# dalek-cryptography/curve25519-dalek

Measured on AMD Instinct MI355X. Metric: MSM scalar-mults/sec (variable-base Pippenger MSM), higher is better.
Workload: dtype u32 limbs (radix 2^25.5), u64 accumulators

## Files before the change

### curve25519-dalek_amd/csrc/accum.hip

```cpp
#include <hip/hip_runtime.h>
#include <stdlib.h>
#define C25519_CHAIN 1
#include "devio.h"
#include "msm_internal.h"
#include "fe26x.h"
#include "msm_sort.h"
#include "mid_long.h"

namespace c25519 {

#if defined(__HIP_DEVICE_COMPILE__)
#define ge_madd_acc ge_madd_signed_p3_lockstep
#else
#define ge_madd_acc ge_madd_signed_p3
#endif

#ifndef C25519_ACC_WAVES
#define C25519_ACC_WAVES 3
#endif
__device__ __forceinline__ void accumulate_body(const u32 *__restrict__ pts, const u32 *__restrict__ sorted, const u32 *__restrict__ base,
             const u32 *__restrict__ perm, u64 count, u64 n, const msm_geom &g, u32 *__restrict__ buckets, int cont, u32 block, uint4 *stage) {
    const u64 tid = (u64)block * blockDim.x + threadIdx.x;
    const bool in_range = tid < count;
    const u64 gid = in_range ? perm[tid] : 0;
// ... 53 lines not shown
        if (active) acc = ge_madd_acc(acc, pts_from_q(q), neg);
#else
        if (active) {
            const u32 me = (u32)((int)e >> 31), flip = me ^ sgn;
            sgn = me;
            acc = ge_madd_lazy_p3_lockstep(acc, pts_from_q(q), flip);
        }
#endif
        e = e_next;
    }
#undef C25519_COOP_ISSUE
    if (!mine) return;
#if !defined(C25519_ACC_SIGN_SELECT) && defined(__HIP_DEVICE_COMPILE__)
    acc.X = fe_carry(feW(fe_cond_neg(acc.X, sgn))); acc.T = fe_carry(feW(fe_cond_neg(acc.T, sgn)));
#endif
    p40_store(buckets, gid, acc);
}
__global__ void __launch_bounds__(256) __attribute__((amdgpu_waves_per_eu(C25519_ACC_WAVES, C25519_ACC_WAVES)))
k_accumulate(const u32 *__restrict__ pts, const u32 *__restrict__ sorted, const u32 *__restrict__ base,
             const u32 *__restrict__ perm, u64 count, u64 n, msm_geom g, u32 *__restrict__ buckets, int cont) {
    __shared__ uint4 stage[(256 / 64) * 8 * 64];
    accumulate_body(pts, sorted, base, perm, count, n, g, buckets, cont, blockIdx.x, stage);
}
struct acc_long_args { const mid_item *items; const u32 *counters; u32 *seg_sums; u32 *long_done; u32 max_items, blocks; };
__global__ void __launch_bounds__(256) __attribute__((amdgpu_waves_per_eu(C25519_ACC_WAVES, C25519_ACC_WAVES)))
k_accumulate_long(const u32 *__restrict__ pts, const u32 *__restrict__ sorted, const u32 *__restrict__ base,
                  const u32 *__restrict__ perm, u64 count, u64 n, msm_geom g, u32 *__restrict__ buckets, acc_long_args L) {
    __shared__ uint4 stage[(256 / 64) * 8 * 64];
    if (blockIdx.x < L.blocks) {
        C25519_PRIO_LONG();
        mid_long_body<1>(pts, sorted, n, g, buckets, L.max_items, L.items, L.counters, L.seg_sums, L.long_done, blockIdx.x * 4u + (threadIdx.x >> 6), L.blocks * 4u);
        return;
    }
    accumulate_body(pts, sorted, base, perm, count, n, g, buckets, 0, blockIdx.x - L.blocks, stage);
}

}

const char *launch_accumulate(const uint32_t *pts, const uint32_t *sorted, const uint32_t *base, const uint32_t *perm, uint64_t count, uint64_t n, const c25519::msm_geom &g, uint32_t *buckets, int cont, hipStream_t st) {
    using namespace c25519;
    hipLaunchKernelGGL(k_accumulate, dim3((unsigned)((count + 255) / 256)), dim3(256), 0, st, pts, sorted, base, perm, count, n, g, buckets, cont);
    return "c25519::k_accumulate (lockstep field products, wave-cooperative gather)";
}
const char *launch_accumulate_long(const uint32_t *pts, const uint32_t *sorted, const uint32_t *base, const uint32_t *perm, uint64_t count, uint64_t n, const c25519::msm_geom &g, uint32_t *buckets,
                                   const void *items, const uint32_t *counters, uint32_t *seg_sums, uint32_t *long_done, uint32_t max_items, uint32_t long_blocks, hipStream_t st) {
    using namespace c25519;
    acc_long_args L = {(const mid_item *)items, counters, seg_sums, long_done, max_items, long_blocks};
    hipLaunchKernelGGL(k_accumulate_long, dim3((unsigned)((count + 255) / 256) + long_blocks), dim3(256), 0, st, pts, sorted, base, perm, count, n, g, buckets, L);
    return "c25519::k_accumulate_long (mid path: bucket lanes of k_accumulate behind the blocks of the over-long lists)";
}
```

### curve25519-dalek_amd/csrc/msm.hip

```cpp
#include <hip/hip_runtime.h>
#include <algorithm>
#include <stdio.h>
#include <stdlib.h>
#include <string.h>
#include <stdexcept>
#include <string>
#include <vector>
#include "../../include/c25519_hip.h"
#include "devio.h"
#include "sc_sha.h"
#include "sc28.h"
#include "kernels.h"
#include "ctx.h"
#include "msm_internal.h"
#include "msm_sort.h"
#include "host51.h"
#include "ffi.h"
#include "capi_util.h"
#include <functional>

using namespace c25519;

namespace c25519 {

// ... 402 lines not shown
    msm_layout(layout_terms ? layout_terms : n, g);
    for (int i = 0; i < reps; i++) {
        msm_plan pl;
        pl.bad_sticky = nullptr;
        int32_t r = msm_enqueue_sort(ctx, d_scalars, n, g, dslot(ctx, 0), nullptr, pl);
        if (r) return r;
    }
    HIPCHK(hipStreamSynchronize(ctx->stream));
    return C25519_OK;
}

static_assert(C25519_SLOT_U32 == MSM_MAX_WIN * 40 + 16, "slot layout");

int32_t msm_enqueue_acc(c25519_ctx *ctx, const msm_plan &pl, const uint32_t *d_pts, uint32_t *d_slot, hipEvent_t *ring, hipEvent_t wait_acc, bool cont, bool reduce,
                        const uint32_t *d_bad_sticky) {
    const msm_geom &g = pl.g;
    if (pl.n > (1ull << 25)) return bad_arg(ctx, "msm: internal error (a pass of more than 2^25 records)");
    if (pl.sort_stream && pl.sort_stream != ctx->stream) {
        HIPCHK(hipEventRecord(ctx->ev_sort, pl.sort_stream));
        HIPCHK(hipStreamWaitEvent(ctx->stream, ctx->ev_sort, 0));
    }
    hipStream_t st = ctx->stream;
    if (wait_acc) HIPCHK(hipStreamWaitEvent(st, wait_acc, 0));
    HIPCHK(hipEventRecord(ctx->ev_fork, st));
    HIPCHK(hipStreamWaitEvent(ctx->aux, ctx->ev_fork, 0));
    hipLaunchKernelGGL(k_long_segments, dim3(std::min<uint32_t>(pl.max_items, 2048u)), dim3(64), 0, ctx->aux, d_pts, pl.sorted, pl.n, g, pl.items, pl.counters, pl.max_items, pl.segs);
    hipLaunchKernelGGL(k_long_combine, dim3(std::min<uint32_t>(pl.max_long, 1024u)), dim3(64), 0, ctx->aux, pl.base, g, pl.counters, pl.max_items, pl.lgids, pl.lfirst, pl.segs, pl.buckets, cont ? 1 : 0);
    if (ring) HIPCHK(hipEventRecord(ring[0], st));
    static const int coop_reduce = C25519_KNOB("REDUCE_COOP", 1);
    const int groups = (g.ngroups > 1 && reduce && !cont && coop_reduce) ? g.ngroups : 1;
    static const int reduce_main = C25519_KNOB("REDUCE_MAIN", 1);
    const bool red_main = reduce_main && ctx->solo && reduce && !cont && groups == 1 && coop_reduce && !wait_acc;
    for (int q = 0; q < groups; q++) {
        const int k0 = groups > 1 ? g.gstart[q] : 0, k1 = groups > 1 ? g.gstart[q + 1] : g.nwin;
        ctx->kname[0] = launch_accumulate(d_pts, pl.sorted, pl.base, pl.perm + (size_t)k0 * g.half, (uint64_t)(k1 - k0) * g.half, pl.n, g, pl.buckets, cont ? 1 : 0, st);
        if (groups > 1) {
            HIPCHK(hipEventRecord(ctx->ev_grp[q], st));
            HIPCHK(hipStreamWaitEvent(ctx->aux, ctx->ev_grp[q], 0));
            launch_bucket_reduce4(pl.buckets, g, pl.nseg, pl.SW, d_slot, d_bad_sticky ? d_bad_sticky : pl.bad_ws, ctx->aux, k0, k1);
            HIPCHK(hipGetLastError());
        }
    }
    HIPCHK(hipEventRecord(ctx->ev_acc, st));
    if (ring) HIPCHK(hipEventRecord(ring[1], st));
    if (red_main) {
        HIPCHK(hipEventRecord(ctx->ev_join, ctx->aux));
        HIPCHK(hipStreamWaitEvent(st, ctx->ev_join, 0));
        launch_bucket_reduce4(pl.buckets, g, pl.nseg, pl.SW, d_slot, d_bad_sticky ? d_bad_sticky : pl.bad_ws, st);
        HIPCHK(hipGetLastError());
        if (ring) HIPCHK(hipEventRecord(ring[2], st));
        return C25519_OK;
    }
    if (reduce && groups == 1) HIPCHK(hipStreamWaitEvent(ctx->aux, ctx->ev_acc, 0));
    if (groups > 1) {
    } else if (reduce && coop_reduce) {
        launch_bucket_reduce4(pl.buckets, g, pl.nseg, pl.SW, d_slot, d_bad_sticky ? d_bad_sticky : pl.bad_ws, ctx->aux);
        HIPCHK(hipGetLastError());
    } else if (reduce) {
// ... 338 lines not shown
    if (!ahead) {
        if ((r = ctx_reserve(ctx, ctx->tmp_e, std::max(n, n_carve) * PTS_BYTES + 256))) return r;
        d_pts = (uint32_t *)ctx->tmp_e.p;
    } else d_pts = ahead->pts + ahead->offset * (PTS_BYTES / 4);
    hipEvent_t *ring = pass_ring(owner, ctx, 1);
    HIPCHK(hipEventRecord(ring[3], ctx->stream));
    HIPCHK(hipEventRecord(ctx->ev_fork, ctx->stream));
    static const int sweep_early = C25519_KNOB("SWEEP_EARLY", 1);
    const bool early = sweep_early && cont && !wait_in && terms > msm_small_max() && parity >= 0;
    hipEvent_t lists_free = nullptr;
    if (parity >= 0) {
        HIPCHK(hipEventRecord(ctx->ev_lists[parity & 1], ctx->stream));
        if (early) lists_free = sweep_early >= 2 ? ctx->ev_lists[(parity & 1) ^ 1] : ctx->ev_fork;
    }
    if (!early) HIPCHK(hipStreamWaitEvent(ctx->aux, ctx->ev_fork, 0));
    if (!cont && !ctx->direct_seq) slot_init(d_slot, terms, nullptr, ctx->stream, g.c);
    if (terms <= msm_small_max() && g.half <= 64 && g.nwin <= 64 && !cont && reduce && !ahead) {
        if (in_fmt == C25519_FMT_RAW160) return msm_small_pass(ctx, d_scalars, d_points, 0, n, g, d_slot, ring, nullptr, wait_acc);
        if ((r = prep_points(ctx, d_points, n, in_fmt, d_pts, 0, slot_flags(d_slot) + 1))) return r;
        return msm_small_pass(ctx, d_scalars, d_pts, 1, n, g, d_slot, ring, nullptr, wait_acc);
    }
    msm_plan pl;
    pl.bad_sticky = d_bad_sticky;
    static const int serial_sort = C25519_KNOB("PROFILE_SERIAL_SORT", 0);
    static const int sort_first = C25519_KNOB("SORT_FIRST", 0);
    const bool sorted_first = sort_first && !ahead && !serial_sort && !cont && !wait_in;
    if (sorted_first) {
        pl.ev_partition = nullptr;
        if ((r = msm_enqueue_sort(ctx, d_scalars, n, g, d_slot, ctx->aux, pl, nullptr, n_carve, lists_free, sweep_early >= 2 ? parity : -1))) return r;
        if (pl.ev_partition) HIPCHK(hipStreamWaitEvent(ctx->stream, pl.ev_partition, 0));
    }
    if (!ahead) { if ((r = prep_points(ctx, d_points, n, in_fmt, d_pts, 0, slot_flags(d_slot) + 1))) return r; }
    else if (ahead->launch) {
        if ((r = prep_points(ctx, d_points, ahead->n, in_fmt, ahead->pts, 0, slot_flags(d_slot) + 1))) return r;
        HIPCHK(hipEventRecord(ahead->done, ctx->stream));
    } else HIPCHK(hipStreamWaitEvent(ctx->stream, ahead->done, 0));
    if (serial_sort) { HIPCHK(hipEventRecord(ctx->ev_z, ctx->stream)); HIPCHK(hipStreamWaitEvent(ctx->aux, ctx->ev_z, 0)); }
    if (!sorted_first && (r = msm_enqueue_sort(ctx, d_scalars, n, g, d_slot, ctx->aux, pl, nullptr, n_carve, lists_free, sweep_early >= 2 ? parity : -1))) return r;
    if (cont && pl.buckets != ctx->cont_buckets) return bad_arg(ctx, "msm: internal error (the workspace of a continuing pass moved its buckets)");
    ctx->cont_buckets = pl.buckets;
    if ((r = msm_enqueue_acc(ctx, pl, d_pts, d_slot, ring, wait_acc, cont, reduce, d_bad_sticky))) return r;
    return C25519_OK;
}
typedef std::function<int32_t(uint64_t lo, uint64_t m, hipEvent_t *ready)> msm_fetch;
static int32_t msm_record_enqueue(c25519_ctx *ctx, const uint8_t *d_scalars, const uint8_t *d_points, uint64_t n, int in_fmt, uint32_t *d_record,
                                  const msm_fetch *fetch = nullptr, uint64_t pass_terms = 0) {
// ... 251 lines not shown
```

### curve25519-dalek_amd/csrc/msm_internal.h

```cpp
#pragma once
#include <hip/hip_runtime.h>
#include <stdint.h>
#include <stdlib.h>
#include "ge26.h"
#include "ctx.h"

#include "knobs.h"
namespace c25519 {
constexpr int MSM_MAX_WIN = 56;
constexpr int MSM_MAX_GROUPS = 4;
struct msm_geom { int c, nwin, half, first_unsigned, bps_log2; u32 long_cap; u32 addk[8]; unsigned char pos[MSM_MAX_WIN], wid[MSM_MAX_WIN], bps[MSM_MAX_WIN];
                  unsigned char ngroups, gstart[MSM_MAX_GROUPS + 1]; };
__host__ __device__ inline int msm_group_of(const msm_geom &g, int k) { int r = 0; for (int i = 1; i < g.ngroups; i++) r += k >= (int)g.gstart[i] ? 1 : 0; return r; }
struct msm_merged { int c, K; uint64_t ns; };
constexpr u32 LONG_CAP_MIN = 192;
constexpr u32 LONG_SEG = 1024;
}
namespace c25519 {
struct long_item;
static inline int red_lb_log2(int half) {
    static const int lb_min = [] { const int v = C25519_KNOB("RED_LB_MIN", 1); return v < 1 ? 1 : (v > 3 ? 3 : v); }();
    if (half <= 512) return 3;
    int lb = lb_min;
    while ((half >> (lb + 6)) > 64) lb++;
    return lb;
}
static inline int red_nseg(int half) { const int seg = 64 << red_lb_log2(half); return (half + seg - 1) / seg; }
constexpr int REC_TERMS_LO = 8, REC_TERMS_HI = 9, REC_PASSES = 10, REC_MAGIC = 11, REC_C = 12;
constexpr u32 REC_MAGIC_VALUE = 0x52503235u;
inline uint64_t msm_small_max() { static const uint64_t v = (uint64_t)C25519_KNOB("MSM_SMALL_MAX", 6143); return v; }
inline uint64_t verify_small_max() { static const uint64_t v = (uint64_t)C25519_KNOB("VERIFY_SMALL_MAX", 4095); return v < msm_small_max() ? v : msm_small_max(); }
inline uint64_t small_upload_max_terms() { static const uint64_t v = (uint64_t)C25519_KNOB_LL("VERIFY_STAGED_MAX", 32769); return v; }
}
static inline unsigned div_up64(uint64_t a, uint64_t b) { return (unsigned)((a + b - 1) / b); }
static inline uint32_t *slot_flags(uint32_t *slot) { return slot + c25519::MSM_MAX_WIN * 40; }
static inline uint32_t *dslot(c25519_ctx *ctx, int i) { return ctx->d_slots + (size_t)i * C25519_SLOT_U32; }
static inline const uint32_t *hslot(c25519_ctx *ctx, int i) { return (const uint32_t *)ctx->h_msm + (size_t)i * C25519_SLOT_U32; }
static inline uint32_t *drec(c25519_ctx *ctx) { return dslot(ctx, C25519_MAX_SLOTS); }
struct msm_plan {
    c25519::msm_geom g; uint64_t n, nb; int nseg; uint32_t max_items, max_long;
    uint32_t *base, *sorted, *buckets, *perm, *SW, *counters, *lgids, *lfirst, *segs, *bad_ws, *bad_sticky = nullptr; c25519::long_item *items;
    hipStream_t sort_stream;
    hipEvent_t ev_partition = nullptr;
};
void msm_sort_params(uint64_t n, c25519::msm_geom &g);
void msm_slice_params(c25519::msm_geom &g);
int32_t msm_enqueue_sort(c25519_ctx *ctx, const uint8_t *d_scalars, uint64_t n_scalars, const c25519::msm_geom &g, uint32_t *d_slot, hipStream_t sort_stream, msm_plan &pl,
                         const c25519::msm_merged *md = nullptr, uint64_t n_carve = 0, hipEvent_t lists_free = nullptr, int parity = -1);
struct msm_matrix_sort_args {
    const uint8_t *d_scalars; uint64_t n_scalars, n; int nchunk; bool use_part; int SL, PART_CHUNK, pchunks;
    uint16_t *D; uint32_t *counts, *P1, *cc, *bin_base, *flags, *totals, *ord_hist;
};
int32_t msm_matrix_sort_enqueue(c25519_ctx *ctx, const c25519::msm_geom &g, const c25519::msm_merged *md, msm_plan &pl, const msm_matrix_sort_args &a, hipStream_t st);
int32_t msm_enqueue_acc(c25519_ctx *ctx, const msm_plan &pl, const uint32_t *d_pts, uint32_t *d_slot, hipEvent_t *ring, hipEvent_t wait_acc, bool cont = false, bool reduce = true,
                        const uint32_t *d_bad_sticky = nullptr);
struct mid_run;
int32_t msm_enqueue(c25519_ctx *ctx, const uint8_t *d_scalars, uint64_t n, const uint32_t *d_pts, const c25519::msm_geom &g, uint32_t *d_slot, hipEvent_t *ring,
                    hipStream_t sort_stream, hipEvent_t wait_acc = nullptr, const struct mid_run *run = nullptr);
int32_t msm_small_enqueue(c25519_ctx *ctx, const uint8_t *d_scalars, const void *d_points, int src_fmt, uint64_t n, const c25519::msm_geom &g, uint32_t *d_slot, hipStream_t st);
c25519::ge_p3 host_p40(const uint32_t *t);
c25519::ge_p3 msm_horner(const uint32_t *cols, const c25519::msm_geom &g);
int32_t slots_collect(c25519_ctx *ctx, int count);
int32_t rec_collect(c25519_ctx *ctx);
void slot_init(uint32_t *d_slot, uint64_t terms, const uint32_t *d_pre, hipStream_t st, int c);
int32_t records_fold(const uint8_t *records, uint64_t count, c25519::ge_p3 &R, uint32_t flags[8], std::string *err);
struct pass_set { c25519_ctx *c[4]; int lanes; };
int32_t passes_begin(c25519_ctx *ctx, uint64_t passes, pass_set &ps);
int32_t passes_join(c25519_ctx *ctx, pass_set &ps);
hipEvent_t *pass_ring(c25519_ctx *owner, c25519_ctx *c, uint8_t kind);
void launch_merged_table(const uint8_t *in_raw, uint64_t ns, int c, int K, uint8_t *out_raw, hipStream_t st);
void launch_bucket_reduce4(const uint32_t *buckets, const c25519::msm_geom &g, int nseg, uint32_t *SW, uint32_t *d_slot, const uint32_t *bad_ws, hipStream_t st, int k0 = 0, int k1 = -1);
void msm_set_groups(c25519::msm_geom &g, int groups, int last);
namespace c25519 { struct reduce_publish { int on; uint32_t *host_flag; uint32_t seq, terms_lo, terms_hi, c; int hdr; const uint32_t *dev_flags; }; }
void launch_bucket_reduce_pub(const uint32_t *buckets, const c25519::msm_geom &g, int nseg, uint32_t *SW, uint32_t *out, const uint32_t *blockflags, int nflags, uint32_t *done_cnt,
                              const c25519::reduce_publish &pub, hipStream_t st);
void launch_order_place(const uint32_t *totals, uint64_t nb, const uint32_t *ord_hist, uint32_t *ord_cursor, uint32_t *perm, const c25519::msm_geom &g, hipStream_t st);
uint64_t msm_mid_max();
bool msm_mid_serves_terms(uint64_t n);
bool msm_mid_serves(uint64_t n, const c25519::msm_geom &g, bool prepared);
struct mid_run { hipStream_t stream; hipEvent_t recs_ready; const uint8_t *sign_z16; uint64_t sign_first, sign_count; };
int32_t msm_mid_enqueue(c25519_ctx *ctx, const uint8_t *d_scalars, const void *points, int src_fmt, uint64_t n, const c25519::msm_geom &g, uint32_t *d_slot, int hdr, uint64_t terms, hipEvent_t *ring,
                        const mid_run *run = nullptr);
void launch_apply_sign(uint32_t *pts, uint64_t dst0, const uint8_t *z16, uint64_t n, hipStream_t st);
void launch_prep_basepoint(uint32_t *pts, uint64_t dst, hipStream_t st);
void launch_record_sum(uint32_t *rec, const uint32_t *slots, int cnt, int nwin, int first, hipStream_t st);
const char *launch_accumulate(const uint32_t *pts, const uint32_t *sorted, const uint32_t *base, const uint32_t *perm, uint64_t count, uint64_t n, const c25519::msm_geom &g, uint32_t *buckets, int cont, hipStream_t st);
const char *launch_accumulate_long(const uint32_t *pts, const uint32_t *sorted, const uint32_t *base, const uint32_t *perm, uint64_t count, uint64_t n, const c25519::msm_geom &g, uint32_t *buckets,
                                   const void *items, const uint32_t *counters, uint32_t *seg_sums, uint32_t *long_done, uint32_t max_items, uint32_t long_blocks, hipStream_t st);
void msm_layout(uint64_t n, c25519::msm_geom &g, int cmax = 0, int c_exact = 0);
int32_t msm_core(c25519_ctx *ctx, const uint8_t *d_scalars, uint64_t n, const uint32_t *d_pts, c25519::ge_p3 &R);
void msm_merged_layout(uint64_t ns, c25519::msm_merged &m);
int32_t msm_merged_core(c25519_ctx *ctx, const uint8_t *d_scalars, uint64_t n, const c25519::msm_merged &m, const uint32_t *d_table, c25519::ge_p3 &R);
int32_t msm_merged_build(c25519_ctx *ctx, const uint8_t *d_points, uint64_t ns, int in_fmt, const c25519::msm_merged &m, uint32_t *d_table, uint32_t *d_badcount);
int32_t prep_points(c25519_ctx *ctx, const uint8_t *d_points, uint64_t n, int in_fmt, uint32_t *d_pts, uint64_t dst0, uint32_t *d_badcount, bool expect_affine = false);
int32_t prep_points_on(c25519_ctx *ctx, const uint8_t *d_points, uint64_t n, int in_fmt, uint32_t *d_pts, uint64_t dst0, uint32_t *d_badcount, hipStream_t st, devbuf &pre, bool expect_affine = false);
void host_encode(const c25519::ge_p3 &R, int out_fmt, uint8_t *out);
void host_raw160(const c25519::ge_p3 &p, uint8_t *out);
c25519::ge_p3 host_from_raw160(const uint8_t *in);
```

### curve25519-dalek_amd/csrc/msm_sort.h

```cpp
#pragma once
#include <hip/hip_runtime.h>
#include "devio.h"
#include "msm_internal.h"

#ifndef C25519_PRIO
#define C25519_PRIO 1
#endif
#if defined(__HIP_DEVICE_COMPILE__) && C25519_PRIO
#define C25519_PRIO_CHAIN() __builtin_amdgcn_s_setprio(3)
#define C25519_PRIO_SIDE() __builtin_amdgcn_s_setprio(2)
#ifndef C25519_PRIO_LONG_LEVEL
#define C25519_PRIO_LONG_LEVEL 2
#endif
#define C25519_PRIO_LONG() __builtin_amdgcn_s_setprio(C25519_PRIO_LONG_LEVEL)
#else
#define C25519_PRIO_LONG() do { } while (0)
#define C25519_PRIO_CHAIN() do { } while (0)
#define C25519_PRIO_SIDE() do { } while (0)
#endif

namespace c25519 {

__device__ __forceinline__ int digit_of(u32 v, int k, const msm_geom &g) {
    return (k >= g.first_unsigned) ? (v <= (u32)g.half ? (int)v : 0) : (int)v - (1 << (g.wid[k] - 1));
// ... 3 lines not shown
#ifndef C25519_PART_CAP
#define C25519_PART_CAP 17408
#endif
constexpr int PART_CAP = C25519_PART_CAP;
static inline int part_chunk(int SL) { return SL <= 128 ? 16384 : 15360; }

__host__ __device__ __forceinline__ int part_entry_shift(const msm_geom &g) { return g.bps_log2 > 8 ? 32 - g.bps_log2 : 24; }
__device__ __forceinline__ bool part_entry(u32 v, int k, const msm_geom &g, int bps, u32 t, u32 &slice, u32 &entry) {
    int d = digit_of(v, k, g);
    if (d == 0) return false;
    u32 b = (u32)((d > 0 ? d : -d) - 1);
    const int sh = part_entry_shift(g);
    slice = b >> bps;
    entry = ((b & ((1u << bps) - 1u)) << sh) | (d < 0 ? (1u << (sh - 1)) : 0u) | t;
    return true;
}
__device__ __forceinline__ u32 part_entry_final(u32 ev, int sh) { return (ev & ((1u << (sh - 1)) - 1u)) | ((ev >> (sh - 1)) << 31); }

constexpr int SWEEP_TPT = 8, SWEEP_THREADS = 1024, SWEEP_WAVES = SWEEP_THREADS / 64, SWEEP_CHUNK = SWEEP_THREADS * SWEEP_TPT;
constexpr int P2G_ITER = 48;

struct long_item { u32 gid, lo, hi, first; };
__device__ __forceinline__ void order_note_bucket(u32 c, u64 G, const msm_geom &g, const u32 *__restrict__ base, u32 *h, u32 max_items, long_item *__restrict__ items,
                                                  u32 *__restrict__ counters, u32 *__restrict__ long_gids, u32 *__restrict__ long_first) {
    atomicAdd(&h[255u - (c > 255u ? 255u : c)], 1u);
    if (c > g.long_cap) {
        const int k = (int)(G / g.half), b = (int)(G % g.half);
        const u32 lo = base[(u64)k * (g.half + 1) + b], hi = lo + c;
        const u32 nseg = (c + LONG_SEG - 1) / LONG_SEG;
        const u32 first = atomicAdd(&counters[0], nseg);
        const u32 lb = atomicAdd(&counters[1], 1u);
        long_gids[lb] = (u32)G;
        long_first[lb] = first;
        for (u32 sg = 0; sg < nseg && first + sg < max_items; sg++) {
            long_item it; it.gid = (u32)G; it.lo = lo + sg * LONG_SEG; it.hi = (it.lo + LONG_SEG < hi) ? it.lo + LONG_SEG : hi; it.first = first;
            items[first + sg] = it;
        }
    }
}

}
```

### curve25519-dalek_amd/csrc/msm_sort.hip

```cpp
#include <hip/hip_runtime.h>
#include <algorithm>
#include <stdlib.h>
#include <string.h>
#include <stdexcept>
#include <string>
#include <vector>
#include <functional>
#include "../../include/c25519_hip.h"
#include "devio.h"
#include "sc_sha.h"
#include "sc28.h"
#include "kernels.h"
#include "ctx.h"
#include "msm_internal.h"
#include "msm_sort.h"
#include "ffi.h"
#include "capi_util.h"

using namespace c25519;


namespace c25519 {

struct sweep_regs { u32 s[SWEEP_TPT][8]; };
// ... 28 lines not shown
    C25519_PRIO_CHAIN();
    extern __shared__ u32 sm[];
    constexpr int NW = THREADS / 64, CHUNK = THREADS * SWEEP_TPT;
    u32 *cnt = sm;
    u32 *cur = sm + NW * SL;
    u32 *ls = sm + 2 * NW * SL;
    u32 *stage = ls + SL + 1;
    __shared__ u32 wtot[NW];
    __shared__ u32 sbad;
    const int j = blockIdx.x, nchunk = gridDim.x, w = threadIdx.x >> 6, lane = threadIdx.x & 63;
    if (blockIdx.x == 0) for (int i = threadIdx.x; i < nzero; i += THREADS) zero_words[i] = 0;
    if (threadIdx.x == 0) sbad = 0;
    const int total = NW * SL, ept = total >= THREADS ? total / THREADS : 1;
    const int base = (int)threadIdx.x * ept;
    for (int i = threadIdx.x; i < total; i += THREADS) cnt[i] = 0;
    __syncthreads();
    const u64 lo = (u64)j * CHUNK;
    sweep_regs R;
    sweep_load<THREADS>(scalars, n, lo, g, R, &sbad, nt);
#pragma unroll 1
    for (int k = 0; k < g.nwin; k++) {
        const int wd = g.wid[k], bps = g.bps[k];
        u32 ent[SWEEP_TPT], slc[SWEEP_TPT];
#pragma unroll
        for (int r = 0; r < SWEEP_TPT; r++) {
            const u32 v = sweep_take(R, r, wd);
            slc[r] = 0xffffffffu;
            u32 sl, e;
            if (part_entry(v, k, g, bps, (u32)lo + (u32)r * THREADS + threadIdx.x, sl, e)) {
                slc[r] = sl * NW + ((u32)w ^ ((sl >> 2) & (NW - 1)));
                ent[r] = e;
                atomicAdd(&cnt[slc[r]], 1u);
            }
        }
        __syncthreads();
        u32 v4[4], tsum = 0;
#pragma unroll
        for (int e = 0; e < 4; e++) {
            v4[e] = 0;
            if (e < ept && base + e < total) { v4[e] = cnt[base + e]; cnt[base + e] = 0; }
            tsum += v4[e];
        }
        u32 inc = tsum;
        for (int off = 1; off < 64; off <<= 1) { const u32 x = __shfl_up(inc, off, 64); if (lane >= off) inc += x; }
        if (lane == 63) wtot[w] = inc;
        __syncthreads();
        u32 run = inc - tsum;
#pragma unroll
        for (int q = 0; q < NW; q++) run += q < w ? wtot[q] : 0u;
#pragma unroll
        for (int e = 0; e < 4; e++) {
            if (e < ept && base + e < total) {
                const int idx = base + e;
                cur[idx] = run;
                if ((idx & (NW - 1)) == 0) ls[idx / NW] = run;
                if (idx == total - 1) ls[SL] = run + v4[e];
            }
            run += v4[e];
        }
        __syncthreads();
#pragma unroll
        for (int r = 0; r < SWEEP_TPT; r++)
            if (slc[r] != 0xffffffffu) stage[atomicAdd(&cur[slc[r]], 1u)] = ent[r];
        __syncthreads();
        const u32 tot = ls[SL];
        u32 *dst = P1 + (u64)k * wstride + (u64)j * CHUNK;
        for (u32 i = threadIdx.x; i < tot; i += THREADS) dst[i] = stage[i];
        for (int i = threadIdx.x; i <= SL; i += THREADS) lsg[((u64)k * (SL + 1) + i) * nchunk + j] = ls[i];
    }
    if (threadIdx.x == 0) bad_blk[j] = sbad;
}
__global__ void __launch_bounds__(256) k_bin_totals(const u32 *__restrict__ lsg, int nchunk, int SL, int nbins, u32 *__restrict__ binm, const u32 *__restrict__ bad_blk,
                                                    u32 *__restrict__ bad_ws, u32 *__restrict__ bad_sticky) {
    C25519_PRIO_CHAIN();
    if (blockIdx.x == 0) {
        u32 any = 0;
        for (int i = threadIdx.x; i < nchunk; i += 256) any |= bad_blk[i];
        any = __syncthreads_or((int)any);
        if (threadIdx.x == 0) { *bad_ws = any ? 1u : 0u; if (any && bad_sticky) atomicOr(bad_sticky, 1u); }
    }
    const int bin = blockIdx.x * 4 + (threadIdx.x >> 6), lane = threadIdx.x & 63;
    if (bin >= nbins) return;
    const int k = bin / SL, s = bin % SL;
    const u32 *row0 = lsg + ((u64)k * (SL + 1) + s) * nchunk, *row1 = row0 + nchunk;
    u32 sum = 0;
    for (int j = lane; j < nchunk; j += 64) sum += row1[j] - row0[j];
#pragma unroll
    for (int d = 32; d > 0; d >>= 1) sum += (u32)__shfl_xor((int)sum, d, 64);
    if (lane == 0) binm[bin] = sum;
}


template <int NW, int ITER>
__global__ void __launch_bounds__(64 * NW) __attribute__((amdgpu_waves_per_eu(NW / 2, NW / 2)))
k_part2g(const u32 *__restrict__ P1, u64 n, u64 wstride, u32 chunk, msm_geom g, int SL, int nchunk, const u32 *__restrict__ lsg, const u32 *__restrict__ binm,
         u32 *__restrict__ totals, u32 *__restrict__ base, u32 *__restrict__ sorted,
         u32 *__restrict__ ord_hist, u32 max_items, long_item *__restrict__ items, u32 *__restrict__ counters,
         u32 *__restrict__ long_gids, u32 *__restrict__ long_first) {
    C25519_PRIO_CHAIN();
    extern __shared__ u32 sm[];
    u32 *cnt = sm, *cur = sm + PART_BPS_MAX, *oh = sm + 2 * PART_BPS_MAX, *out = sm + 3 * PART_BPS_MAX, *wl = out + PART_CAP;
    __shared__ u32 red[NW], red_all[NW];
    const int k = blockIdx.x, sidx = blockIdx.y, tid = threadIdx.x, lane = tid & 63, w = tid >> 6;
    const int PART_BPS = 1 << g.bps[k], sh = part_entry_shift(g);
    const u32 *row0 = lsg + ((u64)k * (SL + 1) + sidx) * nchunk, *row1 = row0 + nchunk;
    const u32 *src = P1 + (u64)k * wstride;
    const u32 mine = tid < SL ? binm[(u64)k * SL + tid] : 0u;
    u32 part = tid < sidx ? mine : 0u, all = mine;
    const u32 m = binm[(u64)k * SL + sidx];
    if (tid < PART_BPS) cnt[tid] = 0;
    if (tid < 256) oh[tid] = 0;
    int nslots = 0;
    for (int j0 = 0; j0 < nchunk; j0 += NW * 64) {
        const int j = j0 + w + NW * lane;
        u32 st = 0, len = 0;
        if (j < nchunk) { st = row0[j]; len = row1[j] - st; }
        const u32 np = (len + 63u) >> 6;
        u32 inc = np;
        for (int off = 1; off < 64; off <<= 1) { const u32 x = __shfl_up(inc, off, 64); if (lane >= off) inc += x; }
        const u32 first = (u32)nslots + inc - np;
        for (u32 p = 0; p < np; p++)
// ... 31 lines not shown
    } else {
        for (int j = w; j < nchunk; j += NW) {
            const u32 st = row0[j], en = row1[j];
            for (u32 o = st + lane; o < en; o += 64) atomicAdd(&cnt[src[(u64)j * chunk + o] >> sh], 1u);
        }
    }
    __syncthreads();
    if (tid < 64) {
        const int per = PART_BPS >> 6;
        u32 c4[8] = {0, 0, 0, 0, 0, 0, 0, 0}, sum = 0;
        for (int q = 0; q < per; q++) { c4[q] = cnt[per * tid + q]; sum += c4[q]; }
        u32 inc = sum;
        for (int off = 1; off < 64; off <<= 1) { u32 x = __shfl_up(inc, off, 64); if (tid >= off) inc += x; }
        u32 run = inc - sum;
        for (int q = 0; q < per; q++) { cur[per * tid + q] = run; run += c4[q]; }
    }
    __syncthreads();
    if (tid < PART_BPS) {
        const u64 b = (u64)sidx * PART_BPS + tid;
        totals[(u64)k * g.half + b] = cnt[tid];
        base[(u64)k * (g.half + 1) + b] = b0 + cur[tid];
    }
    __syncthreads();
    if (tid < PART_BPS) order_note_bucket(cnt[tid], (u64)k * g.half + (u64)sidx * PART_BPS + tid, g, base, oh, max_items, items, counters, long_gids, long_first);
    __syncthreads();
    if (tid < 256 && oh[tid]) atomicAdd(&ord_hist[256 * msm_group_of(g, k) + tid], oh[tid]);
    if (fits) {
#pragma unroll 1
        for (int t0 = 0; t0 < nslots; t0 += 8) {
            u32 ev[8];
            bool ok[8];
#pragma unroll
            for (int q = 0; q < 8; q++) {
                const u32 d = t0 + q < nslots ? wl[w * ITER + t0 + q] : 0u;
                ok[q] = (u32)lane < (d & 127u);
                ev[q] = ok[q] ? src[(d >> 7) + lane] : 0u;
            }
#pragma unroll
            for (int q = 0; q < 8; q++) if (ok[q]) out[atomicAdd(&cur[ev[q] >> sh], 1u)] = part_entry_final(ev[q], sh);
        }
        __syncthreads();
        for (u32 i = tid; i < m; i += 64 * NW) dst[i] = out[i];
    } else {
        for (int j = w; j < nchunk; j += NW) {
            const u32 st = row0[j], en = row1[j];
            for (u32 o0 = st; o0 < en; o0 += 64) {
                const u32 o = o0 + lane;
// ... 77 lines not shown
                         const msm_merged *md, uint64_t n_carve, hipEvent_t lists_free, int parity) {
    (void)d_slot;
    const uint64_t n = md ? (uint64_t)md->K * md->ns : n_scalars;
    const uint64_t nc = n_carve > n ? n_carve : n;
    if (!md && (g.half < 64 || n > (1ull << (part_entry_shift(g) - 1)))) return bad_arg(ctx, "msm: internal error (a pass outside the range of the chunk-local sort)");
    static const uint64_t chunk_local_min = (uint64_t)C25519_KNOB("SORT_CHUNK_LOCAL_MIN", 1 << 16);
    const bool matrix = md != nullptr || nc < chunk_local_min;
    int nchunk = std::max(1, std::min(64, 512 / g.nwin));
    while (nchunk > 1 && nc / nchunk < 4096) nchunk /= 2;
    if ((nc + nchunk - 1) / nchunk > 65536) nchunk = (int)((nc + 65535) / 65536);
    const uint64_t nb = (uint64_t)g.nwin * g.half;
    const int nseg = red_nseg(g.half);
    size_t off = 0;
    auto carve = [&](size_t bytes) { size_t o = off; off += (bytes + 255) & ~(size_t)255; return o; };
    const int copies = parity >= 0 ? 2 : 1, cp = parity >= 0 ? (parity & 1) : 0;
    const size_t szB = ((size_t)g.nwin * (g.half + 1) * 4 + 255) & ~(size_t)255, szS = ((size_t)g.nwin * nc * 4 + 255) & ~(size_t)255, szPerm = (nb * 4 + 255) & ~(size_t)255;
    const size_t oD = carve(matrix ? (size_t)g.nwin * nc * 2 : 0), oC = carve(matrix ? (size_t)g.nwin * nchunk * g.half * 4 : 0), oB = carve(szB * copies) + szB * cp;
    const size_t oS = carve(szS * copies) + szS * cp, oK = carve(nb * 160), oT = carve(nb * 4);
    const size_t oSW = carve((size_t)g.nwin * nseg * 2 * 160), oF = carve(16384), oPerm = carve(szPerm * copies) + szPerm * cp;
    const uint64_t entries = (uint64_t)g.nwin * nc;
    const uint32_t max_long = (uint32_t)std::min<uint64_t>(nb, entries / g.long_cap + 1);
    const uint32_t max_items = (uint32_t)(entries / LONG_SEG + max_long + 1);
    const size_t oLI = carve((size_t)max_items * sizeof(long_item)), oLG = carve((size_t)max_long * 4), oLF = carve((size_t)max_long * 4);
    const size_t oLS = carve((size_t)max_items * 160);
    const bool use_part = matrix && g.c >= 13 && n <= (1ull << 23) && n >= (1ull << 16);
    static const int small_blocks = C25519_KNOB("SORT_SMALL", 0);
    static const int sweep_threads = small_blocks ? 256 : (C25519_KNOB("SWEEP_THREADS", SWEEP_THREADS) == 512 ? 512 : SWEEP_THREADS);
    const int sweep_chunk = sweep_threads * SWEEP_TPT;
    const int SL = std::max(1, g.half >> g.bps_log2), PART_CHUNK = matrix ? part_chunk(SL) : sweep_chunk, pchunks = (int)((n + PART_CHUNK - 1) / PART_CHUNK), pchunks_c = (int)((nc + PART_CHUNK - 1) / PART_CHUNK);
    const size_t p1_words = matrix ? (size_t)g.nwin * nc : (size_t)g.nwin * pchunks_c * sweep_chunk;
    size_t oP1 = 0, oCC = 0, oBB = 0;
    if (!matrix || use_part) { oP1 = carve(p1_words * 4); oCC = carve((size_t)g.nwin * (SL + 1) * pchunks_c * 4); oBB = carve((size_t)g.nwin * (SL + 1) * 4 + (size_t)pchunks_c * 4); }
    int32_t r = ctx_reserve(ctx, ctx->tmp_d, off);
    if (r) return r;
    uint8_t *ws = (uint8_t *)ctx->tmp_d.p;
    uint32_t *base = (uint32_t *)(ws + oB), *sorted = (uint32_t *)(ws + oS), *buckets = (uint32_t *)(ws + oK);
    uint32_t *flags = (uint32_t *)(ws + oF), *totals = (uint32_t *)(ws + oT), *ord_hist = flags + 64, *perm = (uint32_t *)(ws + oPerm);
    const int ngr = g.ngroups > 1 ? g.ngroups : 1;
    uint32_t *ord_cursor = flags + 64 + 256 * ngr, *bad_ws = flags + 64 + 512 * ngr;
    const int ZERO_WORDS = 64 + 512 * ngr;
    if (ngr > 1 && (matrix || g.half < 1024)) return bad_arg(ctx, "msm: internal error (window groups outside the chunk-local sort)");
    pl.g = g; pl.n = n; pl.nb = nb; pl.nseg = nseg; pl.max_items = max_items; pl.max_long = max_long;
    pl.base = base; pl.sorted = sorted; pl.buckets = buckets; pl.perm = perm; pl.SW = (uint32_t *)(ws + oSW); pl.counters = flags + 8; pl.bad_ws = bad_ws;
    pl.items = (long_item *)(ws + oLI); pl.lgids = (uint32_t *)(ws + oLG); pl.lfirst = (uint32_t *)(ws + oLF); pl.segs = (uint32_t *)(ws + oLS);
    pl.sort_stream = sort_stream;
    hipStream_t st = sort_stream ? sort_stream : ctx->stream;
    if (matrix) {
        if (lists_free) HIPCHK(hipStreamWaitEvent(st, lists_free, 0));
        msm_matrix_sort_args a;
        a.d_scalars = d_scalars; a.n_scalars = n_scalars; a.n = n; a.nchunk = nchunk; a.use_part = use_part; a.SL = SL; a.PART_CHUNK = PART_CHUNK; a.pchunks = pchunks;
        a.D = (uint16_t *)(ws + oD); a.counts = (uint32_t *)(ws + oC); a.P1 = (uint32_t *)(ws + oP1); a.cc = (uint32_t *)(ws + oCC); a.bin_base = (uint32_t *)(ws + oBB);
        a.flags = flags; a.totals = totals; a.ord_hist = ord_hist;
        return msm_matrix_sort_enqueue(ctx, g, md, pl, a, st);
    }
    uint32_t *P1 = (uint32_t *)(ws + oP1), *lsg = (uint32_t *)(ws + oCC), *binm = (uint32_t *)(ws + oBB), *bad_blk = binm + (size_t)g.nwin * (SL + 1);
    const uint64_t wstride = (uint64_t)pchunks_c * sweep_chunk;
    constexpr int ITER_SMALL = 160;
    const int nw1 = sweep_chunk / SWEEP_TPT / 64;
    const size_t lds1 = ((size_t)2 * nw1 * SL + SL + 1 + sweep_chunk) * 4;
    const size_t lds2 = ((size_t)3 * PART_BPS_MAX + PART_CAP + (small_blocks ? 8 * ITER_SMALL : 16 * P2G_ITER)) * 4;
    static const int sweep_nt = C25519_KNOB("SWEEP_NT", 0);
    if (small_blocks) {
        HIPCHK(hipFuncSetAttribute(reinterpret_cast<const void *>(k_sweep_local<256>), hipFuncAttributeMaxDynamicSharedMemorySize, (int)lds1));
        HIPCHK(hipFuncSetAttribute(reinterpret_cast<const void *>(k_part2g<8, ITER_SMALL>), hipFuncAttributeMaxDynamicSharedMemorySize, (int)lds2));
        hipLaunchKernelGGL(k_sweep_local<256>, dim3(pchunks), dim3(256), lds1, st, d_scalars, n, g, SL, lsg, bad_blk, P1, wstride, flags, ZERO_WORDS, sweep_nt);
    } else if (sweep_threads == 512) {
        HIPCHK(hipFuncSetAttribute(reinterpret_cast<const void *>(k_part2g<16, P2G_ITER>), hipFuncAttributeMaxDynamicSharedMemorySize, (int)lds2));
        hipLaunchKernelGGL(k_sweep_local<512>, dim3(pchunks), dim3(512), lds1, st, d_scalars, n, g, SL, lsg, bad_blk, P1, wstride, flags, ZERO_WORDS, sweep_nt);
    } else {
        HIPCHK(hipFuncSetAttribute(reinterpret_cast<const void *>(k_sweep_local<SWEEP_THREADS>), hipFuncAttributeMaxDynamicSharedMemorySize, (int)lds1));
        HIPCHK(hipFuncSetAttribute(reinterpret_cast<const void *>(k_part2g<16, P2G_ITER>), hipFuncAttributeMaxDynamicSharedMemorySize, (int)lds2));
        hipLaunchKernelGGL(k_sweep_local<SWEEP_THREADS>, dim3(pchunks), dim3(SWEEP_THREADS), lds1, st, d_scalars, n, g, SL, lsg, bad_blk, P1, wstride, flags, ZERO_WORDS, sweep_nt);
    }
    hipLaunchKernelGGL(k_bin_totals, dim3((g.nwin * SL + 3) / 4), dim3(256), 0, st, lsg, pchunks, SL, g.nwin * SL, binm, bad_blk, bad_ws, pl.bad_sticky);
    if (pl.ev_partition) HIPCHK(hipEventRecord(pl.ev_partition, st));
    if (lists_free) HIPCHK(hipStreamWaitEvent(st, lists_free, 0));
    if (small_blocks) hipLaunchKernelGGL((k_part2g<8, ITER_SMALL>), dim3(g.nwin, SL), dim3(512), lds2, st, P1, n, wstride, (u32)sweep_chunk, g, SL, pchunks, lsg, binm, totals, base, sorted, ord_hist, max_items, pl.items, pl.counters, pl.lgids, pl.lfirst);
    else hipLaunchKernelGGL((k_part2g<16, P2G_ITER>), dim3(g.nwin, SL), dim3(1024), lds2, st, P1, n, wstride, (u32)sweep_chunk, g, SL, pchunks, lsg, binm, totals, base, sorted, ord_hist, max_items, pl.items, pl.counters, pl.lgids, pl.lfirst);
    hipLaunchKernelGGL(k_order_place<1024>, dim3(div_up64(nb, 1024)), dim3(1024), 0, st, totals, nb, ord_hist, ord_cursor, perm, g);
    HIPCHK(hipGetLastError());
    return C25519_OK;
}
```

Before: 1.315 billion.

## Fuse long-bucket segment accumulation into the accumulate kernel with completion counters

The separate long-segment and long-combine kernels, which ran on the aux stream behind an event fork, are replaced by a fused launch when there is a single window group. Leading blocks of k_accumulate_long now sum each segment of an over-long bucket list. The last segment to finish, detected through per-bucket atomic done counters, combines the partial sums into the bucket. Separately, the sweep kernel records each entry's rank from the counting atomicAdd, so the scatter pass no longer needs a second atomic per entry. Counters and done flags are now reset inside the sort kernels, which adds some atomics and fences and changes the long-list scheduling.

```diff
diff --git a/curve25519-dalek_amd/csrc/accum.hip b/curve25519-dalek_amd/csrc/accum.hip
--- a/curve25519-dalek_amd/csrc/accum.hip
+++ b/curve25519-dalek_amd/csrc/accum.hip
@@ -99,21 +99,76 @@
     __shared__ uint4 stage[(256 / 64) * 8 * 64];
     accumulate_body(pts, sorted, base, perm, count, n, g, buckets, cont, blockIdx.x, stage);
 }
-struct acc_long_args { const mid_item *items; const u32 *counters; u32 *seg_sums; u32 *long_done; u32 max_items, blocks; };
+struct acc_long_args { const mid_item *items; const u32 *counters; u32 *seg_sums; u32 *long_done; u32 max_items, blocks; const long_item *pitems; int cont; };
+__device__ __forceinline__ void acc_long_body(const u32 *__restrict__ pts, const u32 *__restrict__ sorted, const u32 *__restrict__ base, u64 n, const msm_geom &g, u32 *__restrict__ buckets,
+                                              const acc_long_args &L, u32 wv, u32 nwv) {
+    const u32 nitems = L.counters[0] < L.max_items ? L.counters[0] : L.max_items;
+    const u32 lane = threadIdx.x & 63u;
+#pragma unroll 1
+    for (u32 item = wv; item < nitems; item += nwv) {
+        u32 gid, lo, hi;
+        if (L.pitems) { const long_item it = L.pitems[item]; gid = it.gid; lo = it.lo; hi = it.hi; }
+        else { const mid_item it = L.items[item]; gid = it.gid; lo = it.lo; hi = it.hi; }
+        const u32 *list = sorted + (u64)(gid / (u32)g.half) * n;
+        ge_p3 acc = ge_identity();
+#pragma unroll 1
+        for (u32 i = lo + lane; i < hi; i += 64) {
+            const u32 e = list[i];
+            mid_rec<1> r;
+            r.load(pts, e & 0x7fffffffu);
+            acc = r.add_to(acc, (e >> 31) != 0);
+        }
+        acc = mid_wave_sum(acc);
+        u32 first, done_at, nseg;
+        if (L.pitems) {
+            first = done_at = L.pitems[item].first;
+            const u64 at = (u64)(gid / (u32)g.half) * (g.half + 1) + gid % (u32)g.half;
+            nseg = (base[at + 1] - base[at] + LONG_SEG - 1) / LONG_SEG;
+        } else { const mid_item it = L.items[item]; first = it.first; done_at = it.lb; nseg = it.nseg; }
+        u32 last = 0;
+        if (lane == 0) {
+            p40_store(L.seg_sums, item, acc);
+            __threadfence();
+            last = atomicAdd(&L.long_done[done_at], 1u) == nseg - 1u ? 1u : 0u;
+        }
+        last = (u32)__shfl((int)last, 0, 64);
+        if (last) {
+            __threadfence();
+            ge_p3 tot = ge_identity();
+            bool any = false;
+#pragma unroll 1
+            for (u32 sg = lane; sg < nseg && first + sg < L.max_items; sg += 64) {
+                const ge_p3 v = p40_load(L.seg_sums, first + sg);
+                tot = any ? mid_add_cols(tot, v) : v;
+                any = true;
+            }
+            if (L.cont && lane == 0) tot = mid_add_cols(tot, p40_load(buckets, gid));
+            if (nseg > 1) tot = mid_wave_sum(tot);
+            if (lane == 0) p40_store(buckets, gid, tot);
+        }
+    }
+}
 __global__ void __launch_bounds__(256) __attribute__((amdgpu_waves_per_eu(C25519_ACC_WAVES, C25519_ACC_WAVES)))
 k_accumulate_long(const u32 *__restrict__ pts, const u32 *__restrict__ sorted, const u32 *__restrict__ base,
                   const u32 *__restrict__ perm, u64 count, u64 n, msm_geom g, u32 *__restrict__ buckets, acc_long_args L) {
     __shared__ uint4 stage[(256 / 64) * 8 * 64];
     if (blockIdx.x < L.blocks) {
         C25519_PRIO_LONG();
-        mid_long_body<1>(pts, sorted, n, g, buckets, L.max_items, L.items, L.counters, L.seg_sums, L.long_done, blockIdx.x * 4u + (threadIdx.x >> 6), L.blocks * 4u);
+        acc_long_body(pts, sorted, base, n, g, buckets, L, blockIdx.x * 4u + (threadIdx.x >> 6), L.blocks * 4u);
         return;
     }
-    accumulate_body(pts, sorted, base, perm, count, n, g, buckets, 0, blockIdx.x - L.blocks, stage);
+    accumulate_body(pts, sorted, base, perm, count, n, g, buckets, L.cont, blockIdx.x - L.blocks, stage);
 }
 
 }
 
+const char *launch_accumulate_fused(const uint32_t *pts, const uint32_t *sorted, const uint32_t *base, const uint32_t *perm, uint64_t count, uint64_t n, const c25519::msm_geom &g, uint32_t *buckets, int cont,
+                                    const c25519::long_item *items, const uint32_t *counters, uint32_t *seg_sums, uint32_t *long_done, uint32_t max_items, uint32_t long_blocks, hipStream_t st) {
+    using namespace c25519;
+    acc_long_args L = {nullptr, counters, seg_sums, long_done, max_items, long_blocks, items, cont};
+    hipLaunchKernelGGL(k_accumulate_long, dim3((unsigned)((count + 255) / 256) + long_blocks), dim3(256), 0, st, pts, sorted, base, perm, count, n, g, buckets, L);
+    return "c25519::k_accumulate_long (bucket lanes of k_accumulate behind the blocks of the over-long lists)";
+}
 const char *launch_accumulate(const uint32_t *pts, const uint32_t *sorted, const uint32_t *base, const uint32_t *perm, uint64_t count, uint64_t n, const c25519::msm_geom &g, uint32_t *buckets, int cont, hipStream_t st) {
     using namespace c25519;
     hipLaunchKernelGGL(k_accumulate, dim3((unsigned)((count + 255) / 256)), dim3(256), 0, st, pts, sorted, base, perm, count, n, g, buckets, cont);
@@ -122,7 +177,7 @@
 const char *launch_accumulate_long(const uint32_t *pts, const uint32_t *sorted, const uint32_t *base, const uint32_t *perm, uint64_t count, uint64_t n, const c25519::msm_geom &g, uint32_t *buckets,
                                    const void *items, const uint32_t *counters, uint32_t *seg_sums, uint32_t *long_done, uint32_t max_items, uint32_t long_blocks, hipStream_t st) {
     using namespace c25519;
-    acc_long_args L = {(const mid_item *)items, counters, seg_sums, long_done, max_items, long_blocks};
+    acc_long_args L = {(const mid_item *)items, counters, seg_sums, long_done, max_items, long_blocks, nullptr, 0};
     hipLaunchKernelGGL(k_accumulate_long, dim3((unsigned)((count + 255) / 256) + long_blocks), dim3(256), 0, st, pts, sorted, base, perm, count, n, g, buckets, L);
     return "c25519::k_accumulate_long (mid path: bucket lanes of k_accumulate behind the blocks of the over-long lists)";
 }
diff --git a/curve25519-dalek_amd/csrc/msm.hip b/curve25519-dalek_amd/csrc/msm.hip
--- a/curve25519-dalek_amd/csrc/msm.hip
+++ b/curve25519-dalek_amd/csrc/msm.hip
@@ -448,10 +448,13 @@
     }
     hipStream_t st = ctx->stream;
     if (wait_acc) HIPCHK(hipStreamWaitEvent(st, wait_acc, 0));
-    HIPCHK(hipEventRecord(ctx->ev_fork, st));
-    HIPCHK(hipStreamWaitEvent(ctx->aux, ctx->ev_fork, 0));
-    hipLaunchKernelGGL(k_long_segments, dim3(std::min<uint32_t>(pl.max_items, 2048u)), dim3(64), 0, ctx->aux, d_pts, pl.sorted, pl.n, g, pl.items, pl.counters, pl.max_items, pl.segs);
-    hipLaunchKernelGGL(k_long_combine, dim3(std::min<uint32_t>(pl.max_long, 1024u)), dim3(64), 0, ctx->aux, pl.base, g, pl.counters, pl.max_items, pl.lgids, pl.lfirst, pl.segs, pl.buckets, cont ? 1 : 0);
+    const bool fused = pl.long_done != nullptr && g.ngroups <= 1;
+    if (!fused) {
+        HIPCHK(hipEventRecord(ctx->ev_fork, st));
+        HIPCHK(hipStreamWaitEvent(ctx->aux, ctx->ev_fork, 0));
+        hipLaunchKernelGGL(k_long_segments, dim3(std::min<uint32_t>(pl.max_items, 2048u)), dim3(64), 0, ctx->aux, d_pts, pl.sorted, pl.n, g, pl.items, pl.counters, pl.max_items, pl.segs);
+        hipLaunchKernelGGL(k_long_combine, dim3(std::min<uint32_t>(pl.max_long, 1024u)), dim3(64), 0, ctx->aux, pl.base, g, pl.counters, pl.max_items, pl.lgids, pl.lfirst, pl.segs, pl.buckets, cont ? 1 : 0);
+    }
     if (ring) HIPCHK(hipEventRecord(ring[0], st));
     static const int coop_reduce = C25519_KNOB("REDUCE_COOP", 1);
     const int groups = (g.ngroups > 1 && reduce && !cont && coop_reduce) ? g.ngroups : 1;
@@ -459,7 +462,9 @@
     const bool red_main = reduce_main && ctx->solo && reduce && !cont && groups == 1 && coop_reduce && !wait_acc;
     for (int q = 0; q < groups; q++) {
         const int k0 = groups > 1 ? g.gstart[q] : 0, k1 = groups > 1 ? g.gstart[q + 1] : g.nwin;
-        ctx->kname[0] = launch_accumulate(d_pts, pl.sorted, pl.base, pl.perm + (size_t)k0 * g.half, (uint64_t)(k1 - k0) * g.half, pl.n, g, pl.buckets, cont ? 1 : 0, st);
+        if (fused) ctx->kname[0] = launch_accumulate_fused(d_pts, pl.sorted, pl.base, pl.perm, (uint64_t)g.nwin * g.half, pl.n, g, pl.buckets, cont ? 1 : 0, pl.items, pl.counters, pl.segs, pl.long_done,
+                                                           pl.max_items, std::min<uint32_t>((pl.max_items + 3u) / 4u, 512u), st);
+        else ctx->kname[0] = launch_accumulate(d_pts, pl.sorted, pl.base, pl.perm + (size_t)k0 * g.half, (uint64_t)(k1 - k0) * g.half, pl.n, g, pl.buckets, cont ? 1 : 0, st);
         if (groups > 1) {
             HIPCHK(hipEventRecord(ctx->ev_grp[q], st));
             HIPCHK(hipStreamWaitEvent(ctx->aux, ctx->ev_grp[q], 0));
@@ -844,6 +849,7 @@
     }
     msm_plan pl;
     pl.bad_sticky = d_bad_sticky;
+    pl.fuse_parity = sweep_early < 2 ? parity : -1;
     static const int serial_sort = C25519_KNOB("PROFILE_SERIAL_SORT", 0);
     static const int sort_first = C25519_KNOB("SORT_FIRST", 0);
     const bool sorted_first = sort_first && !ahead && !serial_sort && !cont && !wait_in;
diff --git a/curve25519-dalek_amd/csrc/msm_internal.h b/curve25519-dalek_amd/csrc/msm_internal.h
--- a/curve25519-dalek_amd/csrc/msm_internal.h
+++ b/curve25519-dalek_amd/csrc/msm_internal.h
@@ -41,6 +41,7 @@
     c25519::msm_geom g; uint64_t n, nb; int nseg; uint32_t max_items, max_long;
     uint32_t *base, *sorted, *buckets, *perm, *SW, *counters, *lgids, *lfirst, *segs, *bad_ws, *bad_sticky = nullptr; c25519::long_item *items;
     hipStream_t sort_stream;
+    int fuse_parity = -1; uint32_t *long_done = nullptr;
     hipEvent_t ev_partition = nullptr;
 };
 void msm_sort_params(uint64_t n, c25519::msm_geom &g);
@@ -85,6 +86,8 @@
 void launch_prep_basepoint(uint32_t *pts, uint64_t dst, hipStream_t st);
 void launch_record_sum(uint32_t *rec, const uint32_t *slots, int cnt, int nwin, int first, hipStream_t st);
 const char *launch_accumulate(const uint32_t *pts, const uint32_t *sorted, const uint32_t *base, const uint32_t *perm, uint64_t count, uint64_t n, const c25519::msm_geom &g, uint32_t *buckets, int cont, hipStream_t st);
+const char *launch_accumulate_fused(const uint32_t *pts, const uint32_t *sorted, const uint32_t *base, const uint32_t *perm, uint64_t count, uint64_t n, const c25519::msm_geom &g, uint32_t *buckets, int cont,
+                                    const c25519::long_item *items, const uint32_t *counters, uint32_t *seg_sums, uint32_t *long_done, uint32_t max_items, uint32_t long_blocks, hipStream_t st);
 const char *launch_accumulate_long(const uint32_t *pts, const uint32_t *sorted, const uint32_t *base, const uint32_t *perm, uint64_t count, uint64_t n, const c25519::msm_geom &g, uint32_t *buckets,
                                    const void *items, const uint32_t *counters, uint32_t *seg_sums, uint32_t *long_done, uint32_t max_items, uint32_t long_blocks, hipStream_t st);
 void msm_layout(uint64_t n, c25519::msm_geom &g, int cmax = 0, int c_exact = 0);
diff --git a/curve25519-dalek_amd/csrc/msm_sort.h b/curve25519-dalek_amd/csrc/msm_sort.h
--- a/curve25519-dalek_amd/csrc/msm_sort.h
+++ b/curve25519-dalek_amd/csrc/msm_sort.h
@@ -49,7 +49,7 @@
 
 struct long_item { u32 gid, lo, hi, first; };
 __device__ __forceinline__ void order_note_bucket(u32 c, u64 G, const msm_geom &g, const u32 *__restrict__ base, u32 *h, u32 max_items, long_item *__restrict__ items,
-                                                  u32 *__restrict__ counters, u32 *__restrict__ long_gids, u32 *__restrict__ long_first) {
+                                                  u32 *__restrict__ counters, u32 *__restrict__ long_gids, u32 *__restrict__ long_first, u32 *__restrict__ long_done = nullptr) {
     atomicAdd(&h[255u - (c > 255u ? 255u : c)], 1u);
     if (c > g.long_cap) {
         const int k = (int)(G / g.half), b = (int)(G % g.half);
@@ -59,6 +59,7 @@
         const u32 lb = atomicAdd(&counters[1], 1u);
         long_gids[lb] = (u32)G;
         long_first[lb] = first;
+        if (long_done && first < max_items) long_done[first] = 0;
         for (u32 sg = 0; sg < nseg && first + sg < max_items; sg++) {
             long_item it; it.gid = (u32)G; it.lo = lo + sg * LONG_SEG; it.hi = (it.lo + LONG_SEG < hi) ? it.lo + LONG_SEG : hi; it.first = first;
             items[first + sg] = it;
diff --git a/curve25519-dalek_amd/csrc/msm_sort.hip b/curve25519-dalek_amd/csrc/msm_sort.hip
--- a/curve25519-dalek_amd/csrc/msm_sort.hip
+++ b/curve25519-dalek_amd/csrc/msm_sort.hip
@@ -74,15 +74,16 @@
     for (int k = 0; k < g.nwin; k++) {
         const int wd = g.wid[k], bps = g.bps[k];
         u32 ent[SWEEP_TPT], slc[SWEEP_TPT];
+        static_assert(CHUNK <= (1 << 13), "rank field of the packed slice word");
 #pragma unroll
         for (int r = 0; r < SWEEP_TPT; r++) {
             const u32 v = sweep_take(R, r, wd);
             slc[r] = 0xffffffffu;
             u32 sl, e;
             if (part_entry(v, k, g, bps, (u32)lo + (u32)r * THREADS + threadIdx.x, sl, e)) {
-                slc[r] = sl * NW + ((u32)w ^ ((sl >> 2) & (NW - 1)));
+                const u32 ci = sl * NW + ((u32)w ^ ((sl >> 2) & (NW - 1)));
                 ent[r] = e;
-                atomicAdd(&cnt[slc[r]], 1u);
+                slc[r] = ci | (atomicAdd(&cnt[ci], 1u) << 12);
             }
         }
         __syncthreads();
@@ -113,7 +114,7 @@
         __syncthreads();
 #pragma unroll
         for (int r = 0; r < SWEEP_TPT; r++)
-            if (slc[r] != 0xffffffffu) stage[atomicAdd(&cur[slc[r]], 1u)] = ent[r];
+            if (slc[r] != 0xffffffffu) stage[cur[slc[r] & 0xfffu] + (slc[r] >> 12)] = ent[r];
         __syncthreads();
         const u32 tot = ls[SL];
         u32 *dst = P1 + (u64)k * wstride + (u64)j * CHUNK;
@@ -123,9 +124,10 @@
     if (threadIdx.x == 0) bad_blk[j] = sbad;
 }
 __global__ void __launch_bounds__(256) k_bin_totals(const u32 *__restrict__ lsg, int nchunk, int SL, int nbins, u32 *__restrict__ binm, const u32 *__restrict__ bad_blk,
-                                                    u32 *__restrict__ bad_ws, u32 *__restrict__ bad_sticky) {
+                                                    u32 *__restrict__ bad_ws, u32 *__restrict__ bad_sticky, u32 *__restrict__ long_counters) {
     C25519_PRIO_CHAIN();
     if (blockIdx.x == 0) {
+        if (long_counters && threadIdx.x < 4) long_counters[threadIdx.x] = 0;
         u32 any = 0;
         for (int i = threadIdx.x; i < nchunk; i += 256) any |= bad_blk[i];
         any = __syncthreads_or((int)any);
@@ -148,7 +150,7 @@
 k_part2g(const u32 *__restrict__ P1, u64 n, u64 wstride, u32 chunk, msm_geom g, int SL, int nchunk, const u32 *__restrict__ lsg, const u32 *__restrict__ binm,
          u32 *__restrict__ totals, u32 *__restrict__ base, u32 *__restrict__ sorted,
          u32 *__restrict__ ord_hist, u32 max_items, long_item *__restrict__ items, u32 *__restrict__ counters,
-         u32 *__restrict__ long_gids, u32 *__restrict__ long_first) {
+         u32 *__restrict__ long_gids, u32 *__restrict__ long_first, u32 *__restrict__ long_done) {
     C25519_PRIO_CHAIN();
     extern __shared__ u32 sm[];
     u32 *cnt = sm, *cur = sm + PART_BPS_MAX, *oh = sm + 2 * PART_BPS_MAX, *out = sm + 3 * PART_BPS_MAX, *wl = out + PART_CAP;
@@ -226,7 +228,7 @@
         base[(u64)k * (g.half + 1) + b] = b0 + cur[tid];
     }
     __syncthreads();
-    if (tid < PART_BPS) order_note_bucket(cnt[tid], (u64)k * g.half + (u64)sidx * PART_BPS + tid, g, base, oh, max_items, items, counters, long_gids, long_first);
+    if (tid < PART_BPS) order_note_bucket(cnt[tid], (u64)k * g.half + (u64)sidx * PART_BPS + tid, g, base, oh, max_items, items, counters, long_gids, long_first, long_done);
     __syncthreads();
     if (tid < 256 && oh[tid]) atomicAdd(&ord_hist[256 * msm_group_of(g, k) + tid], oh[tid]);
     if (fits) {
@@ -350,7 +352,7 @@
     const uint32_t max_long = (uint32_t)std::min<uint64_t>(nb, entries / g.long_cap + 1);
     const uint32_t max_items = (uint32_t)(entries / LONG_SEG + max_long + 1);
     const size_t oLI = carve((size_t)max_items * sizeof(long_item)), oLG = carve((size_t)max_long * 4), oLF = carve((size_t)max_long * 4);
-    const size_t oLS = carve((size_t)max_items * 160);
+    const size_t oLS = carve((size_t)max_items * 160), oLD = carve((size_t)max_items * 4);
     const bool use_part = matrix && g.c >= 13 && n <= (1ull << 23) && n >= (1ull << 16);
     static const int small_blocks = C25519_KNOB("SORT_SMALL", 0);
     static const int sweep_threads = small_blocks ? 256 : (C25519_KNOB("SWEEP_THREADS", SWEEP_THREADS) == 512 ? 512 : SWEEP_THREADS);
@@ -381,6 +383,9 @@
         a.flags = flags; a.totals = totals; a.ord_hist = ord_hist;
         return msm_matrix_sort_enqueue(ctx, g, md, pl, a, st);
     }
+    const bool fuse = pl.fuse_parity >= 0;
+    pl.long_done = nullptr;
+    if (fuse) { pl.counters = flags + 4000 + 4 * (pl.fuse_parity & 1); pl.long_done = (uint32_t *)(ws + oLD); }
     uint32_t *P1 = (uint32_t *)(ws + oP1), *lsg = (uint32_t *)(ws + oCC), *binm = (uint32_t *)(ws + oBB), *bad_blk = binm + (size_t)g.nwin * (SL + 1);
     const uint64_t wstride = (uint64_t)pchunks_c * sweep_chunk;
     constexpr int ITER_SMALL = 160;
@@ -400,11 +405,11 @@
         HIPCHK(hipFuncSetAttribute(reinterpret_cast<const void *>(k_part2g<16, P2G_ITER>), hipFuncAttributeMaxDynamicSharedMemorySize, (int)lds2));
         hipLaunchKernelGGL(k_sweep_local<SWEEP_THREADS>, dim3(pchunks), dim3(SWEEP_THREADS), lds1, st, d_scalars, n, g, SL, lsg, bad_blk, P1, wstride, flags, ZERO_WORDS, sweep_nt);
     }
-    hipLaunchKernelGGL(k_bin_totals, dim3((g.nwin * SL + 3) / 4), dim3(256), 0, st, lsg, pchunks, SL, g.nwin * SL, binm, bad_blk, bad_ws, pl.bad_sticky);
+    hipLaunchKernelGGL(k_bin_totals, dim3((g.nwin * SL + 3) / 4), dim3(256), 0, st, lsg, pchunks, SL, g.nwin * SL, binm, bad_blk, bad_ws, pl.bad_sticky, fuse ? pl.counters : nullptr);
     if (pl.ev_partition) HIPCHK(hipEventRecord(pl.ev_partition, st));
     if (lists_free) HIPCHK(hipStreamWaitEvent(st, lists_free, 0));
-    if (small_blocks) hipLaunchKernelGGL((k_part2g<8, ITER_SMALL>), dim3(g.nwin, SL), dim3(512), lds2, st, P1, n, wstride, (u32)sweep_chunk, g, SL, pchunks, lsg, binm, totals, base, sorted, ord_hist, max_items, pl.items, pl.counters, pl.lgids, pl.lfirst);
-    else hipLaunchKernelGGL((k_part2g<16, P2G_ITER>), dim3(g.nwin, SL), dim3(1024), lds2, st, P1, n, wstride, (u32)sweep_chunk, g, SL, pchunks, lsg, binm, totals, base, sorted, ord_hist, max_items, pl.items, pl.counters, pl.lgids, pl.lfirst);
+    if (small_blocks) hipLaunchKernelGGL((k_part2g<8, ITER_SMALL>), dim3(g.nwin, SL), dim3(512), lds2, st, P1, n, wstride, (u32)sweep_chunk, g, SL, pchunks, lsg, binm, totals, base, sorted, ord_hist, max_items, pl.items, pl.counters, pl.lgids, pl.lfirst, pl.long_done);
+    else hipLaunchKernelGGL((k_part2g<16, P2G_ITER>), dim3(g.nwin, SL), dim3(1024), lds2, st, P1, n, wstride, (u32)sweep_chunk, g, SL, pchunks, lsg, binm, totals, base, sorted, ord_hist, max_items, pl.items, pl.counters, pl.lgids, pl.lfirst, pl.long_done);
     hipLaunchKernelGGL(k_order_place<1024>, dim3(div_up64(nb, 1024)), dim3(1024), 0, st, totals, nb, ord_hist, ord_cursor, perm, g);
     HIPCHK(hipGetLastError());
     return C25519_OK;
```

Result: slower. 1.263 billion (-3.9%).
